# laboshinl/loam_velodyne

Hardware: AMD Instinct MI355X
Metric: sweeps/sec (64-ring, 1M-pt map): feature extraction + odometry + scan-to-map registration (higher is better)
Workload: dtype f32

## Files before the change

include/loamx.h:

```cpp
#ifndef LOAMX_H
#define LOAMX_H

#include <stddef.h>
#include <stdint.h>

#ifdef __cplusplus
extern "C" {
#endif

#define LOAMX_OK 0
#define LOAMX_SKIPPED 1
#define LOAMX_E_INVALID (-1)
#define LOAMX_E_CAPACITY (-2)
#define LOAMX_E_HIP (-3)
#define LOAMX_E_NOGPU (-4)
#define LOAMX_E_UNSUPPORTED (-5)
#define LOAMX_E_INTERNAL (-6)

typedef struct loamx_cloud {
  void* data;
  uint32_t count;
  uint32_t stride;
  uint32_t intensity_offset;
  uint32_t reserved;
// ... 36 lines not shown
  uint32_t n_scan_rings;
} loamx_multiscan_mapper;
int loamx_multiscan_mapper_preset(const char* sensor , loamx_multiscan_mapper* out);
int loamx_scanreg_process_raw(loamx_scanreg* h, const loamx_multiscan_mapper* mapper, const void* raw_xyz, uint32_t count,
                              uint32_t stride, loamx_cloud* full, uint32_t* ring_size, loamx_cloud* sharp, loamx_cloud* less_sharp,
                              loamx_cloud* flat, loamx_cloud* less_flat);

enum { LOAMX_RING_FROM_BOUNDS = 0, LOAMX_RING_FROM_TABLE = 1, LOAMX_RING_FROM_FIELD = 2 };
enum { LOAMX_TIME_FROM_AZIMUTH = 0, LOAMX_TIME_FROM_FIELD = 1 };
enum { LOAMX_FIELD_U8 = 1, LOAMX_FIELD_U16 = 2, LOAMX_FIELD_U32 = 3, LOAMX_FIELD_F32 = 4, LOAMX_FIELD_F64 = 5 };
typedef struct loamx_sensor_model {
  uint32_t n_scan_rings;
  uint32_t ring_source, time_source;
  float lower_bound_deg, upper_bound_deg;
  const float* ring_angles_deg;
  float max_angle_error_deg;
  uint32_t ring_offset, ring_type;
  uint32_t time_offset, time_type;
  double time_scale;
} loamx_sensor_model;
int loamx_sensor_model_from_mapper(const loamx_multiscan_mapper* m, loamx_sensor_model* out);
int loamx_sensor_model_check(const loamx_sensor_model* m, uint32_t stride);
int loamx_scanreg_process_sensor(loamx_scanreg* h, const loamx_sensor_model* m, const void* records, uint32_t count, uint32_t stride,
                                 loamx_cloud* full, uint32_t* ring_size, loamx_cloud* sharp, loamx_cloud* less_sharp,
                                 loamx_cloud* flat, loamx_cloud* less_flat);

int loamx_scanreg_update_imu(loamx_scanreg* h, double stamp_sec, float roll, float pitch, float yaw, const float acc_xyz[3]);
int loamx_scanreg_set_time(loamx_scanreg* h, double scan_time_sec);
int loamx_scanreg_get_imu_trans(loamx_scanreg* h, float imu_trans[12]);

typedef struct loamx_odom loamx_odom;

typedef struct loamx_odom_config {
  float scan_period;
  int max_iterations;
  float delta_t_abort;
  float delta_r_abort;
  int device;
} loamx_odom_config;

void loamx_odom_default_config(loamx_odom_config* cfg);
loamx_odom* loamx_odom_create(const loamx_odom_config* cfg);
void loamx_odom_destroy(loamx_odom* h);
int loamx_odom_update_imu(loamx_odom* h, const float imu_trans[12]);
int loamx_odom_process(loamx_odom* h, const loamx_cloud* sharp, const loamx_cloud* less_sharp, const loamx_cloud* flat,
                       const loamx_cloud* less_flat);
int loamx_odom_get_transform(loamx_odom* h, float transform[6]);
int loamx_odom_get_transform_sum(loamx_odom* h, float transform_sum[6]);
int loamx_odom_set_transform(loamx_odom* h, const float transform[6]);
int loamx_odom_set_transform_sum(loamx_odom* h, const float transform_sum[6]);
int loamx_odom_get_last_clouds(loamx_odom* h, loamx_cloud* last_corner, loamx_cloud* last_surf);
int loamx_odom_transform_to_end(loamx_odom* h, loamx_cloud* cloud);
int loamx_odom_get_stats(loamx_odom* h, int stats[4]);

int loamx_scanreg_process_linked(loamx_scanreg* h, const loamx_cloud* cloud, const uint32_t* ring_size, uint32_t n_rings);
int loamx_odom_process_linked(loamx_odom* h, loamx_scanreg* sr);
int loamx_odom_link_wait(loamx_odom* h);

typedef struct loamx_map loamx_map;

typedef struct loamx_map_config {
  float scan_period;
  int max_iterations;
  float delta_t_abort;
  float delta_r_abort;
  float corner_filter_size;
  float surf_filter_size;
  float map_filter_size;
  int device;
} loamx_map_config;

void loamx_map_default_config(loamx_map_config* cfg);
loamx_map* loamx_map_create(const loamx_map_config* cfg);
void loamx_map_destroy(loamx_map* h);
int loamx_map_update_odometry(loamx_map* h, const float transform_sum[6]);
int loamx_map_process(loamx_map* h, const loamx_cloud* corner_last, const loamx_cloud* surf_last, loamx_cloud* full_res);
int loamx_map_process_linked(loamx_map* h, loamx_odom* od, loamx_cloud* full_res_registered);
int loamx_map_get_speculation(loamx_map* h, uint64_t counts[2]);
int loamx_map_insert(loamx_map* h, const loamx_cloud* corner_last, const loamx_cloud* surf_last, const float pose6[6]);
int loamx_map_get_transform(loamx_map* h, int which, float transform[6]);
int loamx_map_set_transform(loamx_map* h, int which, const float transform[6]);
int loamx_map_update_imu(loamx_map* h, double stamp_sec, float roll, float pitch);
int loamx_map_set_time(loamx_map* h, double laser_odometry_time_sec);
int loamx_map_has_fresh_map(loamx_map* h);
int loamx_map_get_surround(loamx_map* h, loamx_cloud* out);
int loamx_map_load_cubes(loamx_map* h, const loamx_cloud* corner, const loamx_cloud* surf);
int loamx_map_get_cubes(loamx_map* h, int which, loamx_cloud* out);
int loamx_map_save_snapshot(loamx_map* h, const char* path);
int loamx_map_load_snapshot(loamx_map* h, const char* path);
int loamx_map_set_timing(loamx_map* h, int on);
int loamx_map_get_timing(loamx_map* h, float ms[4], uint64_t counts[4]);
int loamx_map_get_stats(loamx_map* h, int stats[8]);

typedef struct loamx_tm loamx_tm;
loamx_tm* loamx_tm_create(void);
void loamx_tm_destroy(loamx_tm* h);
int loamx_tm_update_odometry(loamx_tm* h, const float transform_sum[6]);
int loamx_tm_update_mapping_transform(loamx_tm* h, const float aft_mapped[6], const float bef_mapped[6]);
int loamx_tm_associate_to_map(loamx_tm* h);
int loamx_tm_get_mapped(loamx_tm* h, float transform_mapped[6]);
int loamx_wire_pose_to_quat(const float rot_xyz[3], double quat_xyzw[4]);
int loamx_wire_quat_to_pose(const double quat_xyzw[4], float rot_xyz[3]);

typedef struct loamx_batch loamx_batch;

loamx_batch* loamx_batch_create(const loamx_map_config* cfg, uint32_t max_sweeps);
// ... 548 lines not shown
```

loam_velodyne_amd/csrc/api_odom.hip:

```cpp
#include "api_handles.h"

using namespace loamx;

extern "C" {

void loamx_odom_default_config(loamx_odom_config* cfg) {
  if (!cfg) return;
  cfg->scan_period = 0.1f;
  cfg->max_iterations = 25;
  cfg->delta_t_abort = 0.1f;
  cfg->delta_r_abort = 0.1f;
  cfg->device = 0;
}

loamx_odom* loamx_odom_create(const loamx_odom_config* cfg) {
  loamx_odom* h = nullptr;
  guard([&]() {
    loamx_odom_config c;
    if (cfg) c = *cfg; else loamx_odom_default_config(&c);
    LX_REQUIRE(c.scan_period > 0.f, "scan_period must be positive");
    LX_REQUIRE(c.max_iterations >= 1 && c.max_iterations <= 255, "max_iterations must be in [1, 255]");
    LX_REQUIRE(c.delta_t_abort > 0.f && c.delta_r_abort > 0.f, "abort thresholds must be positive");
    h = new loamx_odom(c.device);
    h->od.params.scan_period = c.scan_period;
// ... 19 lines not shown
    LX_REQUIRE(h && sharp && less_sharp && flat && less_flat, "NULL argument");
    return h->od.process_host(sharp, less_sharp, flat, less_flat);
  });
}
int loamx_odom_process_linked(loamx_odom* h, loamx_scanreg* sr) {
  return guard([&]() {
    LX_REQUIRE(h && sr, "NULL argument");
    LX_REQUIRE(sr->fx.device() == h->od.device(), "linked handles must live on one device");
    const float4* p[4] = {nullptr, nullptr, nullptr, nullptr};
    uint32_t n[4] = {0, 0, 0, 0};
    const float4* full = sr->fx.d_cloud() + sr->fx.point_base(0);
    const uint32_t n_full = sr->fx.point_base(1) - sr->fx.point_base(0);
    if (sr->fx.split_results()) {
      sr->fx.device_results_front(0, p, n);
      return h->od.process_linked(p, n, full, n_full, [sr](const float4*& q, uint32_t& c) { sr->fx.device_results_lf(0, q, c); });
    }
    sr->fx.device_results(0, p, n);
    return h->od.process_linked(p, n, full, n_full);
  });
}
int loamx_odom_link_wait(loamx_odom* h) {
  return guard([&]() {
    LX_REQUIRE(h, "NULL handle");
    if (h->od.link_ready()) LX_HIP(hipEventSynchronize(h->od.link_ready()));
    return LOAMX_OK;
  });
}
int loamx_odom_get_transform(loamx_odom* h, float t[6]) {
  return guard([&]() { LX_REQUIRE(h && t, "NULL argument"); h->od.stream_state(0).transform.get(t); return LOAMX_OK; });
}
int loamx_odom_get_transform_sum(loamx_odom* h, float t[6]) {
  return guard([&]() { LX_REQUIRE(h && t, "NULL argument"); h->od.stream_state(0).transform_sum.get(t); return LOAMX_OK; });
}
int loamx_odom_set_transform(loamx_odom* h, const float t[6]) {
  return guard([&]() { LX_REQUIRE(h && t, "NULL argument"); h->od.stream_state(0).transform.set(t); return LOAMX_OK; });
}
int loamx_odom_set_transform_sum(loamx_odom* h, const float t[6]) {
  return guard([&]() { LX_REQUIRE(h && t, "NULL argument"); h->od.stream_state(0).transform_sum.set(t); return LOAMX_OK; });
}
int loamx_odom_get_last_clouds(loamx_odom* h, loamx_cloud* last_corner, loamx_cloud* last_surf) {
  return guard([&]() { LX_REQUIRE(h, "NULL handle"); return h->od.get_last_clouds(0, last_corner, last_surf); });
}
int loamx_odom_transform_to_end(loamx_odom* h, loamx_cloud* cloud) {
  return guard([&]() { LX_REQUIRE(h && cloud, "NULL argument"); return h->od.transform_to_end_host(0, cloud); });
}
int loamx_odom_get_stats(loamx_odom* h, int stats[4]) {
  return guard([&]() {
    LX_REQUIRE(h && stats, "NULL argument");
    OdomStats s = h->od.stream_state(0).stats;
    stats[0] = s.iterations; stats[1] = s.sel; stats[2] = s.frame; stats[3] = s.degenerate;
    return LOAMX_OK;
  });
}

}
```

loam_velodyne_amd/csrc/odometry.hip:

```cpp
#include "odometry.hpp"
#include "odom_schedule.hpp"
#include "pinned_copy.hpp"
#include <chrono>
#include <cstring>
#include <type_traits>

namespace loamx {

constexpr int OD_THREADS = 256;
constexpr int OD_TR_STRIDE = OD_THREADS + 2;
constexpr int OD_PART_STRIDE = 2 * (2 * 16 * LX_NSUM) + 16;
[[maybe_unused]] constexpr int OD_PART_TS = 2 * (2 * 16 * LX_NSUM);

__device__ inline void sincos_f(float a, float& s, float& c) { sincosf(a, &s, &c); }

__device__ inline void transform_to_start(const float* T, float scan_period, const float4 pi, float& x, float& y, float& z) {
  const float s = (1.f / scan_period) * (pi.w - (float)(int)pi.w);
  x = pi.x - s * T[3];
  y = pi.y - s * T[4];
  z = pi.z - s * T[5];
  float sx, cx, sy, cy, sz, cz;
  sincos_f(-s * T[0], sx, cx);
  sincos_f(-s * T[1], sy, cy);
  sincos_f(-s * T[2], sz, cz);
// ... 136 lines not shown
      pos[u] = cc < B.total ? cc + o : B.O[0];
    }
    if (LOAD_FIRST || !first_trip) {
#pragma unroll
      for (int u = 0; u < 4; u++) p[u] = sorted[pos[u]];
      if (LOAD_FIRST && first_trip) {
#pragma unroll
        for (int u = 0; u < OD_BLK_CACHE; u++) first.p[u] = p[u];
      }
    } else {
#pragma unroll
      for (int u = OD_BLK_CACHE; u < 4; u++) p[u] = sorted[pos[u]];
#pragma unroll
      for (int u = 0; u < OD_BLK_CACHE; u++) p[u] = first.p[u];
    }
#pragma unroll
    for (int u = 0; u < 4; u++) visit(p[u], (c0 + 64u * u) < B.total);
  }
}
__device__ inline int nn1_block(const GridDesc& g, const Block27& B, const float4* __restrict__ sorted, const uint32_t* __restrict__ cell_start,
                                float qx, float qy, float qz, int lane, uint32_t& w_out, Block27First& first) {
  float lbest = 25.0f;
  uint32_t lw = 0xffffffffu;
  block27_scan<true>(B, sorted, lane, first, [&](const float4& p, bool valid) {
    const float dx = qx - p.x, dy2 = qy - p.y, dz2 = qz - p.z;
    const float d2 = dx * dx + dy2 * dy2 + dz2 * dz2;
    const uint32_t w = __float_as_uint(p.w);
    if (valid && (d2 < lbest || (d2 == lbest && lw != 0xffffffffu && (w & OD_IDX_MASK) < (lw & OD_IDX_MASK)))) { lbest = d2; lw = w; }
  });
  float d = lbest;
  int j = lw == 0xffffffffu ? -1 : (int)(lw & OD_IDX_MASK), o_ = lw == 0xffffffffu ? 0x7fffffff : (int)(lw & OD_IDX_MASK);
  int ring = (int)(lw >> 24);
  {
#pragma unroll
    for (int off = 32; off > 0; off >>= 1) {
      const float od = __shfl_xor(d, off, 64);
      const int oj = __shfl_xor(j, off, 64), oo = __shfl_xor(o_, off, 64), orr = __shfl_xor(ring, off, 64);
      if (od < d || (od == d && oo < o_)) { d = od; j = oj; o_ = oo; ring = orr; }
    }
  }
  const float h = 1.0f / g.inv_h;
  if (j >= 0 && d < 25.0f && d <= h * h) { w_out = ((uint32_t)ring << 24) | (uint32_t)j; return j; }
  const int id = nn1_shells(g, sorted, cell_start, qx, qy, qz, lane, 2, (j >= 0 && d < 25.0f) ? d : 25.0f, (j >= 0 && d < 25.0f) ? j : -1);
  w_out = id == j ? (((uint32_t)ring << 24) | (uint32_t)j) : (0xff000000u | (uint32_t)(id < 0 ? 0 : id));
  return id;
}

#ifdef LOAMX_PROF_CORR
__device__ unsigned long long g_corr_ts[3][16];
#define OC_TS(k) do { if (blockIdx.y == 0 && lane == 0 && ts_slot >= 0) g_corr_ts[ts_slot][k] = wall_clock64(); } while (0)
#else
#define OC_TS(k) do { } while (0)
#endif
__global__ __launch_bounds__(256) OD_CORR_ATTR void k_odom_corr_grid(OdomProblem* __restrict__ probs, OdomParams P, uint32_t* __restrict__ patch_dst, uint4 patch) {
  if (patch_dst && blockIdx.x == 0 && blockIdx.y == 0 && threadIdx.x == 0) { patch_dst[0] = patch.x; patch_dst[1] = patch.y; patch_dst[2] = patch.z; }
  OdomProblem& pb = probs[blockIdx.y];
  if (pb.done) return;
  const int lane = threadIdx.x & 63, wid = threadIdx.x >> 6;
  const int nSharp = (int)pb.n_sharp, nFlat = (int)pb.n_flat;
  int f;
  {
    const int x = (int)(blockIdx.x % 8), j = (int)(blockIdx.x / 8);
    const int sS = (int)((long long)x * nSharp / 8), nS = (int)((long long)(x + 1) * nSharp / 8) - sS;
    const int sF = (int)((long long)x * nFlat / 8), nF = (int)((long long)(x + 1) * nFlat / 8) - sF;
    const int fl = 4 * j + wid;
    if (fl >= nS + nF) return;
    f = fl < nS ? sS + fl : nSharp + sF + (fl - nS);
  }
#ifdef LOAMX_PROF_CORR
  const int ts_slot = f == nSharp / 2 ? 0 : f == nSharp + nFlat / 2 ? 1 : f == nSharp + nFlat - 1 ? 2 : -1;
#endif
  OC_TS(0);
  float T[6];
#pragma unroll
  for (int k = 0; k < 6; k++) T[k] = pb.transform[k];
  const bool corner = f < nSharp;
  const float4 pi = corner ? pb.sharp[f] : pb.flat[f - nSharp];
  const uint32_t* __restrict__ tbl = corner ? pb.rf_corner : pb.rf_surf;
  const int e0 = max((int)pi.w - 8, 0);
  uint32_t tv = 0u, unordered_epoch = 0u;
  if (tbl) {
    if (e0 + lane < OD_RF_N - 1) tv = tbl[e0 + lane];
    unordered_epoch = tbl[OD_RF_N - 1];
  }
  float x, y, z;
  transform_to_start(T, P.scan_period, pi, x, y, z);
  const GridDescB gd = corner ? *pb.lc_desc : *pb.ls_desc;
  const float4* __restrict__ sorted = pb.sorted;
  const uint32_t* __restrict__ cell_start = pb.cell_table + gd.cell_base;
  OC_TS(1);
  Block27 B;
  block27_build(gd.g, cell_start, x, y, z, lane, B);
  OC_TS(2);
  uint32_t wbest = 0u;
  Block27First first;
  const int closest = nn1_block(gd.g, B, sorted, cell_start, x, y, z, lane, wbest, first);
  OC_TS(3);
  if (closest < 0) {
    if (lane == 0) { pb.ind[5 * f] = -1; pb.ind[5 * f + 1] = -1; pb.ind[5 * f + 2] = -1; }
    return;
  }
  const float4* last = corner ? pb.last_corner : pb.last_surf;
  const int nLast = corner ? (int)pb.n_last_corner : (int)pb.n_last_surf;
  const int nCur = corner ? nSharp : nFlat;
  const int bound = nCur < nLast ? nCur : nLast;
  const int cscan = (wbest >> 24) != 255u ? (int)(wbest >> 24) : (int)last[closest].w;
  float d2 = 25.f, d3 = 25.f;
  int j2 = -1, j3 = -1, o2 = 0x7fffffff, o3 = 0x7fffffff;
  auto better = [](float d, int order, float dbest, int obest) { return d < dbest || (d == dbest && obest != 0x7fffffff && order < obest); };

// ... 84 lines not shown
            } else {
              if (ring <= cscan) { if (better(d, order, d2, o2)) { d2 = d; j2 = j; o2 = order; } }
              else { if (better(d, order, d3, o3)) { d3 = d; j3 = j; o3 = order; } }
            }
          }
          if (mb) stop = true;
        }
        baseF += 256;
        stopF = stop || baseF >= bound;
      }
      if (!stopB) {
        bool stop = false;
#pragma unroll
        for (int u = 0; u < 4; u++) {
          if (stop) continue;
          const int j = baseB - 64 * u - lane;
          const bool in = j >= 0;
          const int ring = (int)qb[u].w;
          const bool brk = in && ((double)ring < (double)cscan - 2.5);
          const unsigned long long mb = __ballot(brk);
          const int fb = mb ? __builtin_ctzll(mb) : 64;
          if (in && lane < fb) {
            const float d = sqd(qb[u], x, y, z);
            const int order = 0x40000000 + (closest - 1 - j);
            if (corner) {
              if (ring < cscan && better(d, order, d2, o2)) { d2 = d; j2 = j; o2 = order; }
            } else {
              if (ring >= cscan) { if (better(d, order, d2, o2)) { d2 = d; j2 = j; o2 = order; } }
              else { if (better(d, order, d3, o3)) { d3 = d; j3 = j; o3 = order; } }
            }
          }
          if (mb) stop = true;
        }
        baseB -= 256;
        stopB = stop || baseB < 0;
      }
    }
    wave_argmin(d2, j2, o2);
    if (!corner) wave_argmin(d3, j3, o3);
  }
  OC_TS(6);
  if (lane == 0) {
    pb.ind[5 * f] = closest;
    pb.ind[5 * f + 1] = j2;
    pb.ind[5 * f + 2] = corner ? -1 : j3;
  }
#ifdef LOAMX_PROF_CORR
  if (blockIdx.y == 0 && lane == 0 && ts_slot >= 0) {
    g_corr_ts[ts_slot][7] = wall_clock64();
    g_corr_ts[ts_slot][8] = (unsigned long long)B.total; g_corr_ts[ts_slot][9] = (unsigned long long)via_block;
    g_corr_ts[ts_slot][10] = (unsigned long long)closest; g_corr_ts[ts_slot][11] = (unsigned long long)cscan;
  }
#endif
}

#ifdef LOAMX_PROF_LM
#define LM_TS(k) do { if (blockIdx.x == 0 && blockIdx.y == 0 && tid == 0 && iter == it_begin + 1) pb.part[OD_PART_TS + (k)] = (double)wall_clock64(); } while (0)
#else
#define LM_TS(k) do { } while (0)
#endif
#ifndef OD_LM_WAVES
#define OD_LM_WAVES 3
#endif
#ifndef OD_LM_WAVES_MIN
#define OD_LM_WAVES_MIN 3
#endif
#define OD_LM_ATTR __attribute__((amdgpu_waves_per_eu(OD_LM_WAVES_MIN, OD_LM_WAVES)))
#pragma clang diagnostic push
#pragma clang diagnostic ignored "-Wpass-failed"
template <int OD_FPT>
__global__ __launch_bounds__(OD_THREADS) OD_LM_ATTR void k_odom_lm(OdomProblem* __restrict__ probs, OdomParams P, int iter0, int n_iters) {
  OdomProblem& pb = probs[blockIdx.y];
  if (pb.done) return;
  const unsigned NB = gridDim.x;
  const int tid = threadIdx.x;
  const int nSharp = (int)pb.n_sharp, nFlat = (int)pb.n_flat, nFeat = nSharp + nFlat;
  __shared__ float T[6];
  __shared__ float trig[6];
  __shared__ double red[8][LX_NSUM];
  using TrT = typename std::conditional<OD_FPT == 1, float, double>::type;
  __shared__ TrT tr[LX_NSUM * OD_TR_STRIDE];
  __shared__ int sh_done, sh_degen, sh_abort;
  __shared__ float matP[36];
  __shared__ float ws[216];
  __shared__ double parts[16 * LX_NSUM];
  __shared__ float AtA[36], AtB[6];
  if (tid < 6) {
    T[tid] = pb.transform[tid];
    const double ang = (double)pb.transform[tid >> 1];
    trig[tid] = (float)((tid & 1) ? cos(ang) : sin(ang));
  }
  const unsigned xtag = pb.xchg_epoch << 8;
  if (tid == 0) { sh_done = 0; sh_abort = 0; sh_degen = pb.stats.degenerate; }
  if (tid < 36) matP[tid] = pb.matP[tid];
  __syncthreads();

  float4 fpo[OD_FPT], ft1[OD_FPT], ft2[OD_FPT], ft3[OD_FPT];
  bool fvalid[OD_FPT], fcorner[OD_FPT];
#pragma unroll
  for (int u = 0; u < OD_FPT; u++) {
    const int f = (u * (int)NB + (int)blockIdx.x) * OD_THREADS + tid;
    fvalid[u] = false;
    fcorner[u] = f < nSharp;
    fpo[u] = ft1[u] = ft2[u] = ft3[u] = make_float4(0.f, 0.f, 0.f, 0.f);
    if (f < nFeat) {
      const int i1 = pb.ind[5 * f], i2 = pb.ind[5 * f + 1], i3 = pb.ind[5 * f + 2];
// ... 479 lines not shown
ToEndParams OdometryBatch::to_end_params(uint32_t s, bool enabled) const { return odom_to_end_params(*streams_[s], params.scan_period, enabled); }

void OdometryBatch::to_end_device(uint32_t s, float4* pts, uint32_t n) {
  if (!n) return;
  hipLaunchKernelGGL(k_transform_to_end, dim3((n + 255) / 256), dim3(256), 0, st_, pts, n, to_end_params(s, true));
}

void odom_integrate_pose(OdomStream& S) {
  HAngle rx, ry, rz;
  accumulate_rotation(S.transform_sum.rot_x, S.transform_sum.rot_y, S.transform_sum.rot_z, -S.transform.rot_x,
                      HAngle((float)(-S.transform.rot_y.r * 1.05)), -S.transform.rot_z, rx, ry, rz);
  HVec3 v{S.transform.pos.x - S.imu_shift.x, S.transform.pos.y - S.imu_shift.y, (float)(S.transform.pos.z * 1.05 - S.imu_shift.z)};
  h_rot_zxy(v, rz, rx, ry);
  HVec3 trans{S.transform_sum.pos.x - v.x, S.transform_sum.pos.y - v.y, S.transform_sum.pos.z - v.z};
  plugin_imu_rotation(rx, ry, rz, S.imu_pitch_start, S.imu_yaw_start, S.imu_roll_start, S.imu_pitch_end, S.imu_yaw_end,
                      S.imu_roll_end, rx, ry, rz);
  S.transform_sum.rot_x = rx; S.transform_sum.rot_y = ry; S.transform_sum.rot_z = rz;
  S.transform_sum.pos = trans;
}
void odom_set_imu(OdomStream& S, const float* t) {
  S.imu_pitch_start = HAngle(t[0]); S.imu_yaw_start = HAngle(t[1]); S.imu_roll_start = HAngle(t[2]);
  S.imu_pitch_end = HAngle(t[3]); S.imu_yaw_end = HAngle(t[4]); S.imu_roll_end = HAngle(t[5]);
  S.imu_shift = {t[6], t[7], t[8]};
  S.imu_velo = {t[9], t[10], t[11]};
}
ToEndParams odom_to_end_params(const OdomStream& S, float scan_period, bool enabled) {
  ToEndParams P;
  S.transform.get(P.T);
  const HAngle* ta[3] = {&S.transform.rot_x, &S.transform.rot_y, &S.transform.rot_z};
  const HAngle* sa[3] = {&S.imu_pitch_start, &S.imu_yaw_start, &S.imu_roll_start};
  const HAngle* ea[3] = {&S.imu_pitch_end, &S.imu_yaw_end, &S.imu_roll_end};
  for (int k = 0; k < 3; k++) {
    P.sT[k] = ta[k]->s; P.cT[k] = ta[k]->c;
    P.s_start[k] = sa[k]->s; P.c_start[k] = sa[k]->c;
    P.s_end[k] = ea[k]->s; P.c_end[k] = ea[k]->c;
  }
  P.shift[0] = S.imu_shift.x; P.shift[1] = S.imu_shift.y; P.shift[2] = S.imu_shift.z;
  P.scan_period = scan_period;
  P.enabled = enabled ? 1 : 0;
  return P;
}

struct OdometryBatch::Pass {
  const OdomInput* in;
  int* rc;
  uint32_t ns, K;
  std::vector<OdomInput> in_late;
  bool late_pending = false, patch_pending = false;
  uint32_t n_corner_all = 0, n_all = 0;
  const float4 *src_c = nullptr, *src_s = nullptr;
  std::vector<uint32_t> active;
  uint32_t max_feat = 0, max_sharp = 0, max_flat = 0;
  LtCall* lt = nullptr;
};

void OdometryBatch::process(const OdomInput* in, int* rc, bool defer_tail) {
  TraceRange trace_range("loamx:odometry");
  LX_HIP(hipSetDevice(device_));
  if (up_pending_) {
    LX_HIP(hipEventSynchronize(ev_up_));
    up_pending_ = false;
  }
  Pass p{in, rc, n_streams(), 2 * n_streams()};
  stage_clouds_(p);
  build_problems_(p);
  upload_(p);
  launch_pairs_(p);
  enqueue_tail_(p);
  if (!p.active.empty()) collect_(p);
  integrate_poses_(p);
  if (!defer_tail) {
    LX_HIP(hipStreamSynchronize(st_));
    tail_pending_ = false;
  }
}

void OdometryBatch::stage_clouds_(Pass& p) {
  const uint32_t ns = p.ns;
  p.late_pending = ns == 1 && (bool)late_less_flat;
  if (p.late_pending) {
    p.in_late.assign(p.in, p.in + ns);
    p.in_late[0].less_flat = nullptr; p.in_late[0].n_less_flat = 0;
    p.in = p.in_late.data();
  }
  const OdomInput* in = p.in;
  for (uint32_t s = 0; s < ns; s++) {
    h_cur_off_[s + 1] = h_cur_off_[s] + in[s].n_less_sharp;
    if (s > 0) LX_REQUIRE(in[s].less_sharp == in[s - 1].less_sharp + in[s - 1].n_less_sharp || in[s].n_less_sharp == 0 || in[s - 1].n_less_sharp == 0,
                          "less_sharp clouds of the streams must be contiguous");
  }
  for (uint32_t s = 0; s < ns; s++) h_cur_off_[ns + s + 1] = h_cur_off_[ns + s] + in[s].n_less_flat;
  const uint32_t n_corner_all = p.n_corner_all = h_cur_off_[ns], n_all = p.n_all = h_cur_off_[p.K];
  cur_.reserve((size_t)n_all + (p.late_pending ? late_bound : 0u) + 1);
  bool contig_c = true, contig_s = true;
  for (uint32_t s = 1; s < ns; s++) {
    contig_c = contig_c && in[s].less_sharp == in[s - 1].less_sharp + in[s - 1].n_less_sharp;
    contig_s = contig_s && in[s].less_flat == in[s - 1].less_flat + in[s - 1].n_less_flat;
  }
  if (contig_c && contig_s) { p.src_c = in[0].less_sharp; p.src_s = in[0].less_flat; return; }
  if (contig_c) {
    if (n_corner_all) LX_HIP(hipMemcpyAsync(cur_.p, in[0].less_sharp, sizeof(float4) * n_corner_all, hipMemcpyDeviceToDevice, st_));
  } else {
    for (uint32_t s = 0; s < ns; s++)
      if (in[s].n_less_sharp) LX_HIP(hipMemcpyAsync(cur_.p + h_cur_off_[s], in[s].less_sharp, sizeof(float4) * in[s].n_less_sharp, hipMemcpyDeviceToDevice, st_));
  }
  if (contig_s) {
    if (n_all > n_corner_all) LX_HIP(hipMemcpyAsync(cur_.p + n_corner_all, in[0].less_flat, sizeof(float4) * (n_all - n_corner_all), hipMemcpyDeviceToDevice, st_));
  } else {
    for (uint32_t s = 0; s < ns; s++)
      if (in[s].n_less_flat) LX_HIP(hipMemcpyAsync(cur_.p + h_cur_off_[ns + s], in[s].less_flat, sizeof(float4) * in[s].n_less_flat, hipMemcpyDeviceToDevice, st_));
  }
}

void OdometryBatch::resolve_late_(Pass& p) {
  if (!p.late_pending) return;
  p.late_pending = false;
  const float4* pts = nullptr;
  uint32_t n = 0;
  late_less_flat(pts, n);
  LX_REQUIRE(n <= late_bound, "internal: the late less-flat cloud is larger than its announced bound");
  p.in_late[0].less_flat = pts; p.in_late[0].n_less_flat = n;
  h_cur_off_[p.ns + 1] = h_cur_off_[p.ns] + n;
  p.n_all = h_cur_off_[p.K];
  p.src_s = pts;
  p.patch_pending = true;
}
void OdometryBatch::flush_patch_(Pass& p) {
  if (!p.patch_pending) return;
  p.patch_pending = false;
  h_off_late_.reserve(p.K + 1);
  memcpy(h_off_late_.p, h_cur_off_.data(), sizeof(uint32_t) * (p.K + 1));
  LX_HIP(hipMemcpyAsync(d_cur_off_.p, h_off_late_.p, sizeof(uint32_t) * (p.K + 1), hipMemcpyHostToDevice, st_));
  LX_HIP(hipEventRecord(ev_up_, st_));
}

void OdometryBatch::build_problems_(Pass& p) {
  const uint32_t ns = p.ns;
  xchg_epoch_ = xchg_epoch_ % 0xffffffu + 1u;
  std::vector<uint32_t> ind_off(ns + 1, 0);
  for (uint32_t s = 0; s < ns; s++) ind_off[s + 1] = ind_off[s] + 5 * (p.in[s].n_sharp + p.in[s].n_flat) + 5;
  ind_.reserve(ind_off[ns] + 8);
  for (uint32_t s = 0; s < ns; s++) {
    OdomStream& S = *streams_[s];
    const OdomInput& I = p.in[s];
    if (!S.inited) {
      S.transform_sum.rot_x = HAngle(S.transform_sum.rot_x.r + S.imu_pitch_start.r);
      S.transform_sum.rot_z = HAngle(S.transform_sum.rot_z.r + S.imu_roll_start.r);
      p.rc[s] = LOAMX_SKIPPED;
      continue;
    }
    p.rc[s] = LOAMX_OK;
    S.frame++;
    S.transform.pos.x -= S.imu_velo.x * params.scan_period;
    S.transform.pos.y -= S.imu_velo.y * params.scan_period;
    S.transform.pos.z -= S.imu_velo.z * params.scan_period;
    S.stats = {0, 0, (int)S.frame, 0};
    if (S.n_last_corner > 10 && S.n_last_surf > 100) {
      OdomProblem& pb = h_prob_.p[p.active.size()];
      pb.sharp = I.sharp; pb.n_sharp = I.n_sharp;
      pb.flat = I.flat; pb.n_flat = I.n_flat;
      pb.last_corner = last_.p + h_last_off_[s]; pb.n_last_corner = S.n_last_corner;
      pb.last_surf = last_.p + h_last_off_[ns + s]; pb.n_last_surf = S.n_last_surf;
      pb.sorted = index_.sorted();
      pb.cell_table = index_.cell_table();
      pb.lc_desc = index_.desc(s);
      pb.ls_desc = index_.desc(ns + s);
      pb.ind = ind_.p + ind_off[s];
      S.transform.get(pb.transform);
      pb.stats = {0, 0, 0, 0};
      pb.done = 0;
      pb.ticket = 0;
      pb.xchg_epoch = xchg_epoch_;
      pb.stream_id = (int)s;
      pb.host_mirror = h_mirror_.p + p.active.size();
      pb.te_out = te_.p + s;
      pb.part = part_.p + (size_t)p.active.size() * OD_PART_STRIDE;
      pb.err_word = h_err_.p;
      pb.rf_corner = rf_.p + (size_t)s * OD_RF_N;
      pb.rf_surf = rf_.p + (size_t)(ns + s) * OD_RF_N;
      pb.rf_epoch = rf_epoch_;
      p.max_feat = std::max(p.max_feat, I.n_sharp + I.n_flat);
      p.max_sharp = std::max(p.max_sharp, I.n_sharp);
      p.max_flat = std::max(p.max_flat, I.n_flat);
      p.active.push_back(s);
    }
  }
  if (p.max_feat > 32 * OD_THREADS) throw Error(LOAMX_E_CAPACITY, "more than 8192 sharp+flat features in one sweep");
}

void OdometryBatch::upload_(Pass& p) {
  for (uint32_t s = 0; s < p.ns; s++) h_te_.p[s] = to_end_params(s, p.rc[s] == LOAMX_OK);
  memcpy(h_off_pin_.p, h_cur_off_.data(), sizeof(uint32_t) * (p.K + 1));
  LX_HIP(hipMemcpyAsync(up_dev_.p, up_host_.p, up_bytes_, hipMemcpyHostToDevice, st_));
  index_.prepare(p.K);
  if (!ev_up_) LX_HIP(hipEventCreateWithFlags(&ev_up_, hipEventDisableTiming));
  LX_HIP(hipEventRecord(ev_up_, st_));
  up_pending_ = true;
}

static dim3 odom_corr_grid(uint32_t max_sharp, uint32_t max_flat, uint32_t na) {
  return dim3(8 * (((max_sharp + 7) / 8 + (max_flat + 7) / 8 + 3) / 4), na);
}
OdometryBatch::LmGeometry OdometryBatch::lm_geometry_(uint32_t max_feat) {
#ifdef OD_LM_HALF_WGS
  const uint32_t nb = std::min<uint32_t>(16u, std::max<uint32_t>(1u, (max_feat + 2 * OD_THREADS - 1) / (2 * OD_THREADS)));
#else
  const uint32_t nb = std::min<uint32_t>(16u, (max_feat + OD_THREADS - 1) / OD_THREADS);
#endif
  const bool two = max_feat > nb * OD_THREADS;
  if (!lm_slots_[two]) {
    int per_cu = 0;
    if (two) LX_HIP(hipOccupancyMaxActiveBlocksPerMultiprocessor(&per_cu, k_odom_lm<2>, OD_THREADS, 0));
    else LX_HIP(hipOccupancyMaxActiveBlocksPerMultiprocessor(&per_cu, k_odom_lm<1>, OD_THREADS, 0));
    hipDeviceProp_t prop;
    LX_HIP(hipGetDeviceProperties(&prop, device_));
    lm_slots_[two] = (uint32_t)std::max(per_cu, 1) * (uint32_t)std::max(prop.multiProcessorCount, 1);
  }
  return {nb, two, std::max<uint32_t>(1u, (lm_slots_[two] / 2) / nb)};
}

void OdometryBatch::enqueue_corr_(Pass& p, int k) {
  LtCall* lt = p.lt;
  const int lk = lt && k < LT_MAXP ? k : -1;
  if (lk >= 0) {
    for (int e = 0; e < 3; e++) if (!lt->ev[3 * lk + e]) LX_HIP(hipEventCreate(&lt->ev[3 * lk + e]));
    LX_HIP(hipEventRecord(lt->ev[3 * lk], st_));
  }
  uint32_t* pd = nullptr;
  uint4 pv = make_uint4(0u, 0u, 0u, 0u);
  if (p.patch_pending) { p.patch_pending = false; pd = d_cur_off_.p; pv = make_uint4(h_cur_off_[0], h_cur_off_[1], h_cur_off_[2], 0u); }
  hipLaunchKernelGGL(k_odom_corr_grid, odom_corr_grid(p.max_sharp, p.max_flat, (uint32_t)p.active.size()), dim3(256), 0, st_, prob_.p, params, pd, pv);
  if (lk >= 0) LX_HIP(hipEventRecord(lt->ev[3 * lk + 1], st_));
}
void OdometryBatch::enqueue_lm_(Pass& p, int k) {
  LtCall* lt = p.lt;
  const uint32_t na = (uint32_t)p.active.size();
  const int it0 = 5 * k;
  const int nit = std::min(5, params.max_iterations - it0);
  const int lk = lt && k < LT_MAXP ? k : -1;
  const LmGeometry g = lm_geometry_(p.max_feat);
  for (uint32_t a0 = 0; a0 < na; a0 += g.chunk) {
    const uint32_t nc = std::min(g.chunk, na - a0);
    if (g.two) hipLaunchKernelGGL(k_odom_lm<2>, dim3(g.nb, nc), dim3(OD_THREADS), 0, st_, prob_.p + a0, params, it0, nit);
    else hipLaunchKernelGGL(k_odom_lm<1>, dim3(g.nb, nc), dim3(OD_THREADS), 0, st_, prob_.p + a0, params, it0, nit);
  }
  if (lk >= 0) { LX_HIP(hipEventRecord(lt->ev[3 * lk + 2], st_)); lt->pairs = lk + 1; }
}

struct OdometryBatch::PairOps {
  OdometryBatch& o; Pass& p;
  void corr(int k) { o.enqueue_corr_(p, k); }
  void lm(int k) { o.enqueue_lm_(p, k); }
  void after_first() { o.resolve_late_(p); }
  bool behind(int want) const {
    const volatile OdomProblem* hm = o.h_mirror_.p;
    for (size_t a = 0; a < p.active.size(); a++) if (hm[a].done == 0 && hm[a].stats.iterations < want) return true;
    return false;
  }
  bool converged() const { return !behind(o.params.max_iterations); }
  bool wait_settled(int k) const {
    const int want = std::min(5 * (k + 1), o.params.max_iterations);
    const auto t_in = std::chrono::steady_clock::now();
    for (unsigned spins = 0; behind(want);) {
      if ((++spins & 255u) == 0u && std::chrono::steady_clock::now() - t_in > std::chrono::milliseconds(20)) return false;
      cpu_relax();
    }
    return true;
  }
};

void OdometryBatch::launch_pairs_(Pass& p) {
  const uint32_t na = (uint32_t)p.active.size();
  if (launch_timing_.load(std::memory_order_relaxed) && na && p.max_feat) {
    std::lock_guard<std::mutex> lk(lt_mu_);
    lt_resolve_();
    LtCall& c = lt_[lt_next_ % LT_RING];
    if (!c.pending) { p.lt = &c; lt_next_++; c.pairs = 0; }
  }
  if (!na) return;
  if (p.max_feat) {
    const char* e = getenv("LOAMX_ODOM_PAIRS");
    const OdomPairMode mode = !e ? OdomPairMode::Lag : !strcmp(e, "all") ? OdomPairMode::All : !strcmp(e, "exact") ? OdomPairMode::Exact : !strcmp(e, "lag2") ? OdomPairMode::Lag2 : OdomPairMode::Lag;
// ... 223 lines not shown
```

loam_velodyne_amd/csrc/odometry.hpp:

```cpp
#pragma once
#include "common.h"
#include "host_math.h"
#include "registration.hpp"
#include <atomic>
#include <condition_variable>
#include <functional>
#include <mutex>
#include <thread>

namespace loamx {

struct OdomParams {
  float scan_period = 0.1f;
  int max_iterations = 25;
  float delta_t_abort = 0.1f, delta_r_abort = 0.1f;
};

struct OdomStats {
  int iterations, sel, frame, degenerate;
};

struct ToEndParams;

struct OdomProblem {
  const float4* sharp; uint32_t n_sharp;
  const float4* flat; uint32_t n_flat;
  const float4* last_corner; uint32_t n_last_corner;
  const float4* last_surf; uint32_t n_last_surf;
  const float4* sorted;
  const uint32_t* cell_table;
  const GridDescB* lc_desc;
  const GridDescB* ls_desc;
  int* ind;
  float transform[6];
  OdomStats stats;
  int done;
  float matP[36];
  int stream_id;
  ToEndParams* te_out;
  OdomProblem* host_mirror;
  unsigned ticket;
  unsigned xchg_epoch;
  double* part;
  const uint32_t* rf_corner;
  const uint32_t* rf_surf;
  uint32_t rf_epoch;
  uint32_t* err_word;
};

struct OdomInput {
  const float4* sharp; uint32_t n_sharp;
  const float4* less_sharp; uint32_t n_less_sharp;
  const float4* flat; uint32_t n_flat;
  const float4* less_flat; uint32_t n_less_flat;
};

struct ToEndParams {
  float T[6];
  float sT[3], cT[3];
  float shift[3];
  float s_start[3], c_start[3];
  float s_end[3], c_end[3];
  float scan_period;
  int enabled;
};

constexpr int OD_RF_N = 320;

struct ReprojectProbe {
  int variant;
  float4* pts; uint32_t n;
  const uint32_t* d_off; const uint32_t* h_off; uint32_t K, ns;
  const ToEndParams* d_params; const ToEndParams* h_params;
  const float4* src; const float4* src_s; uint32_t n_corner_all;
  uint32_t* bounds; uint32_t* ring_first; uint32_t rf_epoch;
  const float4* const* table; const uint32_t* sid;
};
void reproject_probe_launch(const ReprojectProbe& a, hipStream_t st);

struct OdomStream {
  bool inited = false;
  long frame = 0;
  HTwist transform, transform_sum;
  HAngle imu_roll_start, imu_pitch_start, imu_yaw_start, imu_roll_end, imu_pitch_end, imu_yaw_end;
  HVec3 imu_shift, imu_velo;
  OdomStats stats = {0, 0, 0, 0};
  uint32_t n_last_corner = 0, n_last_surf = 0;
};

class OdometryBatch {
 public:
  OdometryBatch(int device, uint32_t n_streams, hipStream_t shared_stream = nullptr);
  ~OdometryBatch();
  OdomParams params;
  uint32_t n_streams() const { return (uint32_t)streams_.size(); }
  OdomStream& stream_state(uint32_t s) { return *streams_[s]; }
  hipStream_t stream() const { return st_; }
  void update_imu(uint32_t s, const float* t12);
  void process(const OdomInput* in, int* rc, bool defer_tail = false);
  hipEvent_t tail_event() const { return tail_pending_ ? ev_tail_ : nullptr; }
  void set_keep(int n) { keep_ = n < 2 ? 2 : (n > MAX_KEEP ? MAX_KEEP : n); }
  int process_host(const loamx_cloud* sharp, const loamx_cloud* less_sharp, const loamx_cloud* flat, const loamx_cloud* less_flat);
  int process_linked(const float4* const feat[4], const uint32_t n_feat[4], const float4* d_full, uint32_t n_full,
                     const std::function<void(const float4*&, uint32_t&)>& less_flat_late = nullptr);
  hipEvent_t link_ready() const { return ev_link_; }
  const float4* d_link_full() const { return link_full_.p; }
  uint32_t n_link_full() const { return n_link_full_; }
  bool link_valid() const { return link_valid_; }
  int device() const { return device_; }
  int get_last_clouds(uint32_t s, loamx_cloud* corner, loamx_cloud* surf);
  int transform_to_end_host(uint32_t s, loamx_cloud* cloud);
  void to_end_device(uint32_t s, float4* pts, uint32_t n);
  void to_end_gather(float4* dst, const uint32_t* h_off, const float4* const* src, const ToEndParams* seg_params, uint32_t K,
                     hipStream_t stream);
  ToEndParams to_end_params(uint32_t s, bool enabled) const;
  struct LaunchTotals {
    double lm_ms = 0, lm_noop_ms = 0, corr_ms = 0, corr_noop_ms = 0;
    uint64_t lm_launches = 0, lm_noop_launches = 0, lm_iterations = 0, corr_launches = 0, corr_noop_launches = 0;
    uint64_t lm_bytes = 0, corr_features = 0;
  };
  void set_launch_timing(bool on) { launch_timing_.store(on, std::memory_order_relaxed); }
  LaunchTotals launch_totals();
  const float4* d_last_corner(uint32_t s) const { return last_.p + h_last_off_[s]; }
  const float4* d_last_surf(uint32_t s) const { return last_.p + h_last_off_[n_streams() + s]; }

 private:
  int device_;
  hipStream_t st_ = nullptr;
  bool own_stream_ = false;
  std::vector<OdomStream*> streams_;
  DevBuf<float4> cur_, last_;
  static constexpr int MAX_KEEP = 16;
  DevBuf<float4> older_[MAX_KEEP - 1];
  int keep_ = 2;
  std::vector<uint32_t> h_cur_off_, h_last_off_;
  SubMapIndexBatch index_;
  DevBuf<int> ind_;
  DevBuf<double> part_;
  PinBuf<OdomProblem> h_mirror_;
  PinBuf<uint32_t> h_err_;
  DevBuf<uint32_t> rf_;
  uint32_t rf_epoch_ = 0;
  uint32_t xchg_epoch_ = 0;
  template <class T> struct View { T* p = nullptr; };
  DevBuf<char> up_dev_;
  PinBuf<char> up_host_;
  size_t up_bytes_ = 0;
  View<OdomProblem> prob_, h_prob_;
  View<ToEndParams> te_, h_te_;
  View<uint32_t> d_cur_off_, h_off_pin_;
  PinBuf<uint32_t> h_off_late_;
  std::function<void(const float4*&, uint32_t&)> late_less_flat;
  uint32_t late_bound = 0;
  PinBuf<float4> h_stage_;
  PinBuf<float4> h_last_dl_;
  bool last_dl_valid_ = false;
  DevBuf<float4> up_[4], tmp_cloud_, link_full_;
  uint32_t n_link_full_ = 0;
  bool link_valid_ = false;
  hipEvent_t ev_link_ = nullptr;
  int pred_pairs_ = 5;
  uint32_t lm_slots_[2] = {0, 0};
  hipEvent_t ev_tail_ = nullptr, ev_pose_ = nullptr, ev_up_ = nullptr;
  bool tail_pending_ = false, up_pending_ = false;
  PinBuf<char> h_gather_;
  DevBuf<char> d_gather_;
  static constexpr int LT_RING = 8, LT_MAXP = 8;
  struct LtCall {
    hipEvent_t ev[3 * LT_MAXP] = {};
    int pairs = 0;
    bool pending = false;
    int iters[LT_MAXP] = {};
    uint64_t bytes[LT_MAXP] = {}, feats[LT_MAXP] = {};
  };
  LtCall lt_[LT_RING];
  int lt_next_ = 0;
  std::atomic<bool> launch_timing_{false};
  std::mutex lt_mu_;
  LaunchTotals lt_tot_;
  void lt_resolve_();
  struct Pass;
  struct PairOps;
  struct LmGeometry { uint32_t nb; bool two; uint32_t chunk; };
  void stage_clouds_(Pass& p), build_problems_(Pass& p), upload_(Pass& p), launch_pairs_(Pass& p), enqueue_tail_(Pass& p), collect_(Pass& p);
  void integrate_poses_(const Pass& p);
  void resolve_late_(Pass& p), flush_patch_(Pass& p), enqueue_corr_(Pass& p, int k), enqueue_lm_(Pass& p, int k), prof_print_();
  LmGeometry lm_geometry_(uint32_t max_feat);
};

}
// ... 1 lines not shown
```

loam_velodyne_amd/loamx.py:

```python
from __future__ import annotations

import ctypes as C
import os
import numpy as np

_HERE = os.path.dirname(os.path.abspath(__file__))
LIB_PATH = os.environ.get("LOAMX_LIB") or os.path.join(_HERE, "libloamx.so")

OK, SKIPPED, E_INVALID, E_CAPACITY, E_HIP, E_NOGPU, E_UNSUPPORTED, E_INTERNAL = 0, 1, -1, -2, -3, -4, -5, -6


class Cloud(C.Structure):
    _fields_ = [("data", C.c_void_p), ("count", C.c_uint32), ("stride", C.c_uint32),
                ("intensity_offset", C.c_uint32), ("reserved", C.c_uint32)]


class ScanRegConfig(C.Structure):
    _fields_ = [("scan_period", C.c_float), ("n_feature_regions", C.c_int), ("curvature_region", C.c_int),
                ("max_corner_sharp", C.c_int), ("max_surface_flat", C.c_int), ("less_flat_filter_size", C.c_float),
                ("surface_curvature_threshold", C.c_float), ("device", C.c_int), ("max_corner_less_sharp", C.c_int),
                ("imu_history_size", C.c_int)]


class OdomConfig(C.Structure):
# ... 551 lines not shown
        cl = [cloud_of(a) for a in arrs]
        rc = _check(lib().loamx_odom_process(self.h, C.byref(cl[0]), C.byref(cl[1]), C.byref(cl[2]), C.byref(cl[3])))
        self._sizes = (len(arrs[1]), len(arrs[3]))
        return rc

    def process_linked(self, scanreg):
        rc = _check(lib().loamx_odom_process_linked(self.h, scanreg.h))
        self._sizes = (scanreg._linked_n, scanreg._linked_n)
        return rc

    def link_wait(self):
        return _check(lib().loamx_odom_link_wait(self.h))

    def _t(self, fn):
        t = np.zeros(6, np.float32)
        _check(fn(self.h, t.ctypes.data_as(C.c_void_p)))
        return t

    @property
    def transform(self):
        return self._t(lib().loamx_odom_get_transform)

    @property
    def transform_sum(self):
        return self._t(lib().loamx_odom_get_transform_sum)

    def set_transform(self, t6):
        t = np.ascontiguousarray(t6, np.float32)
        _check(lib().loamx_odom_set_transform(self.h, t.ctypes.data_as(C.c_void_p)))

    def set_transform_sum(self, t6):
        t = np.ascontiguousarray(t6, np.float32)
        _check(lib().loamx_odom_set_transform_sum(self.h, t.ctypes.data_as(C.c_void_p)))

    def last_clouds(self):
        c = np.zeros((max(self._sizes[0], 1), 4), np.float32)
        s = np.zeros((max(self._sizes[1], 1), 4), np.float32)
        cc, sc = cloud_of(c), cloud_of(s)
        _check(lib().loamx_odom_get_last_clouds(self.h, C.byref(cc), C.byref(sc)))
        return c[:cc.count].copy(), s[:sc.count].copy()

    def transform_to_end(self, cloud):
        a = as_points(cloud).copy()
        c = cloud_of(a)
        _check(lib().loamx_odom_transform_to_end(self.h, C.byref(c)))
        return a

    def stats(self):
        s = (C.c_int * 4)()
        _check(lib().loamx_odom_get_stats(self.h, s))
        return dict(iterations=s[0], sel=s[1], frame=s[2], degenerate=s[3])


class LaserMapping:

    def __init__(self, **cfg):
        self._c = _cfg(MapConfig, "loamx_map_default_config", **cfg)
        self.h = C.c_void_p(lib().loamx_map_create(C.byref(self._c)))
        if not self.h:
            raise LoamxError(E_INVALID, lib().loamx_last_error().decode())

    def close(self):
        if getattr(self, "h", None):
            lib().loamx_map_destroy(self.h)
            self.h = None

    __del__ = close

    def update_odometry(self, t6):
        t = np.ascontiguousarray(t6, np.float32)
        _check(lib().loamx_map_update_odometry(self.h, t.ctypes.data_as(C.c_void_p)))

    def update_imu(self, stamp, roll, pitch):
        _check(lib().loamx_map_update_imu(self.h, C.c_double(stamp), C.c_float(roll), C.c_float(pitch)))

    def set_time(self, t):
        _check(lib().loamx_map_set_time(self.h, C.c_double(t)))

    def process(self, corner_last, surf_last, full_res=None, inplace=False):
        c, s = as_points(corner_last), as_points(surf_last)
        cc, sc = cloud_of(c), cloud_of(s)
        if full_res is not None:
            f = as_points(full_res) if inplace else as_points(full_res).copy()
            fc = cloud_of(f)
            rc = _check(lib().loamx_map_process(self.h, C.byref(cc), C.byref(sc), C.byref(fc)))
            return rc, f
        rc = _check(lib().loamx_map_process(self.h, C.byref(cc), C.byref(sc), None))
        return rc, None

    def process_linked(self, odometry, full_out=None):
        if full_out is None:
            return _check(lib().loamx_map_process_linked(self.h, odometry.h, None)), None
        fc = cloud_of(full_out)
        rc = _check(lib().loamx_map_process_linked(self.h, odometry.h, C.byref(fc)))
        return rc, full_out[:fc.count]

    def speculation(self):
        c = (C.c_uint64 * 2)()
        _check(lib().loamx_map_get_speculation(self.h, c))
        return int(c[0]), int(c[1])

    def insert(self, corner_last, surf_last, pose6):
        c, s = as_points(corner_last), as_points(surf_last)
        cc, sc = cloud_of(c), cloud_of(s)
        p = np.ascontiguousarray(pose6, np.float32)
        assert p.shape == (6,)
# ... 1554 lines not shown
```

Measured before the change: 16200.

## Pass odometry problem descriptors as kernel arguments instead of H2D upload

When a batch has at most eight active problems, the per-problem descriptors, to-end parameters and offsets are packed into a large kernel-argument struct. The first correspondence kernel writes them to device memory itself, so the separate host-to-device memcpy and the patch mechanism are skipped. This removes a copy and its latency from the start of each odometry pass, at the cost of a bigger kernel-argument payload and a duplicated fill path. It also reuses the ind_off vector across passes and adds counters plus an environment override for choosing the path.

```diff
diff --git a/include/loamx.h b/include/loamx.h
--- a/include/loamx.h
+++ b/include/loamx.h
@@ -112,6 +112,7 @@
 int loamx_odom_get_last_clouds(loamx_odom* h, loamx_cloud* last_corner, loamx_cloud* last_surf);
 int loamx_odom_transform_to_end(loamx_odom* h, loamx_cloud* cloud);
 int loamx_odom_get_stats(loamx_odom* h, int stats[4]);
+void loamx_odom_head_counts(uint64_t counts[2]);
 
 int loamx_scanreg_process_linked(loamx_scanreg* h, const loamx_cloud* cloud, const uint32_t* ring_size, uint32_t n_rings);
 int loamx_odom_process_linked(loamx_odom* h, loamx_scanreg* sr);
diff --git a/loam_velodyne_amd/csrc/api_odom.hip b/loam_velodyne_amd/csrc/api_odom.hip
--- a/loam_velodyne_amd/csrc/api_odom.hip
+++ b/loam_velodyne_amd/csrc/api_odom.hip
@@ -95,5 +95,8 @@
     return LOAMX_OK;
   });
 }
+void loamx_odom_head_counts(uint64_t counts[2]) {
+  if (counts) odom_head_counts(counts);
+}
 
 }
diff --git a/loam_velodyne_amd/csrc/odometry.hip b/loam_velodyne_amd/csrc/odometry.hip
--- a/loam_velodyne_amd/csrc/odometry.hip
+++ b/loam_velodyne_amd/csrc/odometry.hip
@@ -212,10 +212,7 @@
 #else
 #define OC_TS(k) do { } while (0)
 #endif
-__global__ __launch_bounds__(256) OD_CORR_ATTR void k_odom_corr_grid(OdomProblem* __restrict__ probs, OdomParams P, uint32_t* __restrict__ patch_dst, uint4 patch) {
-  if (patch_dst && blockIdx.x == 0 && blockIdx.y == 0 && threadIdx.x == 0) { patch_dst[0] = patch.x; patch_dst[1] = patch.y; patch_dst[2] = patch.z; }
-  OdomProblem& pb = probs[blockIdx.y];
-  if (pb.done) return;
+template <class PB> __device__ __forceinline__ void odom_corr_grid_body(const PB& pb, const OdomParams& P) {
   const int lane = threadIdx.x & 63, wid = threadIdx.x >> 6;
   const int nSharp = (int)pb.n_sharp, nFlat = (int)pb.n_flat;
   int f;
@@ -406,6 +403,36 @@
     g_corr_ts[ts_slot][10] = (unsigned long long)closest; g_corr_ts[ts_slot][11] = (unsigned long long)cscan;
   }
 #endif
+}
+__global__ __launch_bounds__(256) OD_CORR_ATTR void k_odom_corr_grid(OdomProblem* __restrict__ probs, OdomParams P, uint32_t* __restrict__ patch_dst, uint4 patch) {
+  if (patch_dst && blockIdx.x == 0 && blockIdx.y == 0 && threadIdx.x == 0) { patch_dst[0] = patch.x; patch_dst[1] = patch.y; patch_dst[2] = patch.z; }
+  const OdomProblem& pb = probs[blockIdx.y];
+  if (pb.done) return;
+  odom_corr_grid_body(pb, P);
+}
+__global__ __launch_bounds__(256) OD_CORR_ATTR void k_odom_corr_grid_head(OdomProblem* __restrict__ probs, OdomParams P, OdomHead H) {
+  const OdomHeadProblem& h = H.prob[blockIdx.y];
+  if (blockIdx.x == 0) {
+    const uint32_t t = threadIdx.x;
+    if (t == 0) {
+      OdomProblem o = {};
+      o.sharp = h.sharp; o.n_sharp = h.n_sharp; o.flat = h.flat; o.n_flat = h.n_flat;
+      o.last_corner = h.last_corner; o.n_last_corner = h.n_last_corner; o.last_surf = h.last_surf; o.n_last_surf = h.n_last_surf;
+      o.sorted = h.sorted; o.cell_table = h.cell_table; o.lc_desc = h.lc_desc; o.ls_desc = h.ls_desc;
+      o.ind = h.ind;
+#pragma unroll
+      for (int k = 0; k < 6; k++) o.transform[k] = h.transform[k];
+      o.stream_id = h.stream_id; o.te_out = h.te_out; o.host_mirror = h.host_mirror;
+      o.xchg_epoch = h.xchg_epoch; o.part = h.part;
+      o.rf_corner = h.rf_corner; o.rf_surf = h.rf_surf; o.rf_epoch = h.rf_epoch; o.err_word = h.err_word;
+      probs[blockIdx.y] = o;
+    }
+    if (blockIdx.y == 0) {
+      if (t >= 64 && t - 64 < H.n_te) H.te_dst[t - 64] = H.te[t - 64];
+      if (t >= 128 && t - 128 < H.n_off) H.off_dst[t - 128] = H.off[t - 128];
+    }
+  }
+  odom_corr_grid_body(h, P);
 }
 
 #ifdef LOAMX_PROF_LM
@@ -991,6 +1018,7 @@
   std::vector<uint32_t> active;
   uint32_t max_feat = 0, max_sharp = 0, max_flat = 0;
   LtCall* lt = nullptr;
+  bool head = false;
 };
 
 void OdometryBatch::process(const OdomInput* in, int* rc, bool defer_tail) {
@@ -1070,13 +1098,16 @@
   h_off_late_.reserve(p.K + 1);
   memcpy(h_off_late_.p, h_cur_off_.data(), sizeof(uint32_t) * (p.K + 1));
   LX_HIP(hipMemcpyAsync(d_cur_off_.p, h_off_late_.p, sizeof(uint32_t) * (p.K + 1), hipMemcpyHostToDevice, st_));
+  if (!ev_up_) LX_HIP(hipEventCreateWithFlags(&ev_up_, hipEventDisableTiming));
   LX_HIP(hipEventRecord(ev_up_, st_));
+  up_pending_ = true;
 }
 
 void OdometryBatch::build_problems_(Pass& p) {
   const uint32_t ns = p.ns;
   xchg_epoch_ = xchg_epoch_ % 0xffffffu + 1u;
-  std::vector<uint32_t> ind_off(ns + 1, 0);
+  std::vector<uint32_t>& ind_off = ind_off_;
+  ind_off.assign(ns + 1, 0);
   for (uint32_t s = 0; s < ns; s++) ind_off[s + 1] = ind_off[s] + 5 * (p.in[s].n_sharp + p.in[s].n_flat) + 5;
   ind_.reserve(ind_off[ns] + 8);
   for (uint32_t s = 0; s < ns; s++) {
@@ -1127,8 +1158,20 @@
   if (p.max_feat > 32 * OD_THREADS) throw Error(LOAMX_E_CAPACITY, "more than 8192 sharp+flat features in one sweep");
 }
 
+static std::atomic<uint64_t> g_head_counts[2];
+void odom_head_counts(uint64_t counts[2]) {
+  for (int k = 0; k < 2; k++) counts[k] = g_head_counts[k].load(std::memory_order_relaxed);
+}
+
 void OdometryBatch::upload_(Pass& p) {
   for (uint32_t s = 0; s < p.ns; s++) h_te_.p[s] = to_end_params(s, p.rc[s] == LOAMX_OK);
+  const char* e = getenv("LOAMX_ODOM_HEAD");
+  p.head = !(e && !strcmp(e, "copy")) && !p.active.empty() && p.max_feat > 0 && p.active.size() <= OD_HEAD_MAX && p.ns <= OD_HEAD_MAX;
+  g_head_counts[p.head ? 0 : 1].fetch_add(1, std::memory_order_relaxed);
+  if (p.head) {
+    index_.prepare(p.K);
+    return;
+  }
   memcpy(h_off_pin_.p, h_cur_off_.data(), sizeof(uint32_t) * (p.K + 1));
   LX_HIP(hipMemcpyAsync(up_dev_.p, up_host_.p, up_bytes_, hipMemcpyHostToDevice, st_));
   index_.prepare(p.K);
@@ -1167,6 +1210,30 @@
   }
   uint32_t* pd = nullptr;
   uint4 pv = make_uint4(0u, 0u, 0u, 0u);
+  if (p.head) {
+    p.head = false;
+    p.patch_pending = false;
+    const uint32_t na = (uint32_t)p.active.size();
+    OdomHead H;
+    H.te_dst = te_.p; H.off_dst = d_cur_off_.p;
+    H.n_prob = na; H.n_te = p.ns; H.n_off = p.K + 1;
+    for (uint32_t i = 0; i <= p.K; i++) H.off[i] = h_cur_off_[i];
+    for (uint32_t s = 0; s < p.ns; s++) H.te[s] = h_te_.p[s];
+    for (uint32_t a = 0; a < na; a++) {
+      const OdomProblem& b = h_prob_.p[a];
+      OdomHeadProblem& h = H.prob[a];
+      h.sharp = b.sharp; h.flat = b.flat; h.last_corner = b.last_corner; h.last_surf = b.last_surf;
+      h.sorted = b.sorted; h.cell_table = b.cell_table; h.lc_desc = b.lc_desc; h.ls_desc = b.ls_desc;
+      h.ind = b.ind; h.te_out = b.te_out; h.host_mirror = b.host_mirror; h.part = b.part;
+      h.rf_corner = b.rf_corner; h.rf_surf = b.rf_surf; h.err_word = b.err_word;
+      h.n_sharp = b.n_sharp; h.n_flat = b.n_flat; h.n_last_corner = b.n_last_corner; h.n_last_surf = b.n_last_surf;
+      for (int j = 0; j < 6; j++) h.transform[j] = b.transform[j];
+      h.stream_id = b.stream_id; h.xchg_epoch = b.xchg_epoch; h.rf_epoch = b.rf_epoch;
+    }
+    hipLaunchKernelGGL(k_odom_corr_grid_head, odom_corr_grid(p.max_sharp, p.max_flat, na), dim3(256), 0, st_, prob_.p, params, H);
+    if (lk >= 0) LX_HIP(hipEventRecord(lt->ev[3 * lk + 1], st_));
+    return;
+  }
   if (p.patch_pending) { p.patch_pending = false; pd = d_cur_off_.p; pv = make_uint4(h_cur_off_[0], h_cur_off_[1], h_cur_off_[2], 0u); }
   hipLaunchKernelGGL(k_odom_corr_grid, odom_corr_grid(p.max_sharp, p.max_flat, (uint32_t)p.active.size()), dim3(256), 0, st_, prob_.p, params, pd, pv);
   if (lk >= 0) LX_HIP(hipEventRecord(lt->ev[3 * lk + 1], st_));
diff --git a/loam_velodyne_amd/csrc/odometry.hpp b/loam_velodyne_amd/csrc/odometry.hpp
--- a/loam_velodyne_amd/csrc/odometry.hpp
+++ b/loam_velodyne_amd/csrc/odometry.hpp
@@ -64,6 +64,29 @@
   float scan_period;
   int enabled;
 };
+
+constexpr uint32_t OD_HEAD_MAX = 8;
+struct OdomHeadProblem {
+  const float4* sharp; const float4* flat; const float4* last_corner; const float4* last_surf;
+  const float4* sorted; const uint32_t* cell_table; const GridDescB* lc_desc; const GridDescB* ls_desc;
+  int* ind;
+  ToEndParams* te_out; OdomProblem* host_mirror; double* part;
+  const uint32_t* rf_corner; const uint32_t* rf_surf; uint32_t* err_word;
+  uint32_t n_sharp, n_flat, n_last_corner, n_last_surf;
+  float transform[6];
+  int stream_id;
+  unsigned xchg_epoch;
+  uint32_t rf_epoch;
+};
+struct OdomHead {
+  ToEndParams* te_dst; uint32_t* off_dst;
+  uint32_t n_prob, n_te, n_off;
+  uint32_t off[2 * OD_HEAD_MAX + 1];
+  ToEndParams te[OD_HEAD_MAX];
+  OdomHeadProblem prob[OD_HEAD_MAX];
+};
+static_assert(sizeof(OdomHead) + sizeof(OdomProblem*) + sizeof(OdomParams) + 64 <= 4096, "OdomHead must fit into the kernel arguments");
+void odom_head_counts(uint64_t counts[2]);
 
 constexpr int OD_RF_N = 320;
 
@@ -136,6 +159,7 @@
   std::vector<uint32_t> h_cur_off_, h_last_off_;
   SubMapIndexBatch index_;
   DevBuf<int> ind_;
+  std::vector<uint32_t> ind_off_;
   DevBuf<double> part_;
   PinBuf<OdomProblem> h_mirror_;
   PinBuf<uint32_t> h_err_;
diff --git a/loam_velodyne_amd/loamx.py b/loam_velodyne_amd/loamx.py
--- a/loam_velodyne_amd/loamx.py
+++ b/loam_velodyne_amd/loamx.py
@@ -627,6 +627,12 @@
         return dict(iterations=s[0], sel=s[1], frame=s[2], degenerate=s[3])
 
 
+def odom_head_counts():
+    c = (C.c_uint64 * 2)()
+    lib().loamx_odom_head_counts(c)
+    return int(c[0]), int(c[1])
+
+
 class LaserMapping:
 
     def __init__(self, **cfg):
```

Result: no change. 16100 (median of 2 runs) (-0.6%).
